# AidaDSP/aidadsp-lv2

Measured on AMD Instinct MI355X. Metric: audio samples/sec (48 kHz mono, many streams), higher is better.
Workload: dtype f32; 1 GPU; cfg2: LSTM-32 amp model, 1024 streams/GPU x 256-frame blocks, full run() chain, TTL-default controls; streams_per_gpu=1024, frames=256, kernel=k_lstm_pipe4<32>

## Files before the change

aidadsp-lv2_amd/csrc/aidax_device.h:

```cpp
#pragma once

#include <hip/hip_runtime.h>

#include <cfloat>

#include "aidax_layout.h"

namespace aidax {

__device__ __forceinline__ float dpp_row_shr1(float v)
{
    return __builtin_bit_cast(float, __builtin_amdgcn_update_dpp(0, __builtin_bit_cast(int, v), 0x111, 0xf, 0xf, true));
}

template <int CTRL, int ROW_MASK>
__device__ __forceinline__ float dpp_take(float v)
{
    return __builtin_bit_cast(float, __builtin_amdgcn_update_dpp(0, __builtin_bit_cast(int, v), CTRL, ROW_MASK, 0xf, ROW_MASK == 0xf));
}

__device__ __forceinline__ float wave_sum(float v)
{
    v = v + dpp_take<0xB1, 0xf>(v);
    v = v + dpp_take<0x4E, 0xf>(v);
    v = v + dpp_take<0x141, 0xf>(v);
    v = v + dpp_take<0x140, 0xf>(v);
    v = v + dpp_take<0x142, 0xa>(v);
    v = v + dpp_take<0x143, 0xc>(v);
    return __builtin_bit_cast(float, __builtin_amdgcn_readlane(__builtin_bit_cast(int, v), 63));
}

template <int N>
__device__ __forceinline__ void fmac_row_ror(float& acc, float h, float w)
{
    static_assert(N >= 1 && N <= 15, "rotation within a row of 16 lanes");
    asm volatile("v_fmac_f32_dpp %0, %1, %2 row_ror:%3 row_mask:0xf bank_mask:0xf" : "+v"(acc) : "v"(h), "v"(w), "n"(N));
}

#define AIDAX_ROR1(N, W) "v_fmac_f32_dpp %0, %1, %" #W " row_ror:" #N " row_mask:0xf bank_mask:0xf\n\t"
__device__ __forceinline__ void fmac_row_ror_1_15(float& a0, float h, const float* w)
{
    asm volatile(AIDAX_ROR1(1, 2) AIDAX_ROR1(2, 3) AIDAX_ROR1(3, 4) AIDAX_ROR1(4, 5) AIDAX_ROR1(5, 6) AIDAX_ROR1(6, 7) AIDAX_ROR1(7, 8)
                 AIDAX_ROR1(8, 9) AIDAX_ROR1(9, 10) AIDAX_ROR1(10, 11) AIDAX_ROR1(11, 12) AIDAX_ROR1(12, 13) AIDAX_ROR1(13, 14)
                 AIDAX_ROR1(14, 15) AIDAX_ROR1(15, 16)
                 : "+v"(a0)
                 : "v"(h), "v"(w[1]), "v"(w[2]), "v"(w[3]), "v"(w[4]), "v"(w[5]), "v"(w[6]), "v"(w[7]), "v"(w[8]), "v"(w[9]),
                   "v"(w[10]), "v"(w[11]), "v"(w[12]), "v"(w[13]), "v"(w[14]), "v"(w[15]));
}
#undef AIDAX_ROR1

typedef float aidax_f32x2 __attribute__((ext_vector_type(2)));
#define AIDAX_PKA(ACC, W, HQ) "v_pk_fma_f32 %" #ACC ", %" #W ", %" #HQ ", %" #ACC " op_sel_hi:[1,0,1]\n\t"
#define AIDAX_PKB(ACC, W, HQ) "v_pk_fma_f32 %" #ACC ", %" #W ", %" #HQ ", %" #ACC " op_sel:[0,1,0] op_sel_hi:[1,1,1]\n\t"
#define AIDAX_PKA0(ACC, W, HQ) "v_pk_fma_f32 %" #ACC ", %" #W ", %" #HQ ", 0 op_sel_hi:[1,0,0]\n\t"
#define AIDAX_PKB0(ACC, W, HQ) "v_pk_fma_f32 %" #ACC ", %" #W ", %" #HQ ", 0 op_sel:[0,1,0] op_sel_hi:[1,1,0]\n\t"
__device__ __forceinline__ aidax_f32x2 pk_fma_lds16(aidax_f32x2 pA, const aidax_f32x2* w, const aidax_f32x2* hq)
{
    aidax_f32x2 pB, pC, pD;
    asm volatile(AIDAX_PKA(0, 4, 20) AIDAX_PKB0(1, 5, 20) AIDAX_PKA0(2, 6, 21) AIDAX_PKB0(3, 7, 21)
                 AIDAX_PKA(0, 8, 22) AIDAX_PKB(1, 9, 22) AIDAX_PKA(2, 10, 23) AIDAX_PKB(3, 11, 23)
                 AIDAX_PKA(0, 12, 24) AIDAX_PKB(1, 13, 24) AIDAX_PKA(2, 14, 25) AIDAX_PKB(3, 15, 25)
                 AIDAX_PKA(0, 16, 26) AIDAX_PKB(1, 17, 26) AIDAX_PKA(2, 18, 27) AIDAX_PKB(3, 19, 27)
                 "v_pk_add_f32 %0, %0, %1\n\t"
                 "v_pk_add_f32 %2, %2, %3"
                 : "+v"(pA), "=&v"(pB), "=&v"(pC), "=&v"(pD)
                 : "v"(w[0]), "v"(w[1]), "v"(w[2]), "v"(w[3]), "v"(w[4]), "v"(w[5]), "v"(w[6]), "v"(w[7]), "v"(w[8]), "v"(w[9]), "v"(w[10]),
                   "v"(w[11]), "v"(w[12]), "v"(w[13]), "v"(w[14]), "v"(w[15]),
                   "v"(hq[0]), "v"(hq[1]), "v"(hq[2]), "v"(hq[3]), "v"(hq[4]), "v"(hq[5]), "v"(hq[6]), "v"(hq[7]));
    return pA + pC;
}
#undef AIDAX_PKA
#undef AIDAX_PKB
#undef AIDAX_PKA0
#undef AIDAX_PKB0

struct Pair { float lo, hi; };

__device__ __forceinline__ Pair share_halves(float v)
{
    const unsigned u = __builtin_bit_cast(unsigned, v);
    const auto r = __builtin_amdgcn_permlane32_swap(u, u, false, false);
    const unsigned r0 = r[0], r1 = r[1];
    return { __builtin_bit_cast(float, r0), __builtin_bit_cast(float, r1) };
}

__device__ __forceinline__ Pair share_rows(float v)
{
    const unsigned u = __builtin_bit_cast(unsigned, v);
    const auto r = __builtin_amdgcn_permlane16_swap(u, u, false, false);
    const unsigned r0 = r[0], r1 = r[1];
    return { __builtin_bit_cast(float, r0), __builtin_bit_cast(float, r1) };
}

__device__ __forceinline__ float fast_sigmoid(float v)
{
    const float e = __builtin_amdgcn_exp2f(v * -1.44269504088896340736f);
    return __builtin_amdgcn_rcpf(1.0f + e);
}

constexpr float kNegLog2e = -1.44269504088896340736f;
__device__ __forceinline__ float sigmoid_pre(float v_scaled)
{
    return __builtin_amdgcn_rcpf(1.0f + __builtin_amdgcn_exp2f(v_scaled));
}


constexpr float kTanhP[7] = { 0.9999999933888696f, 0.13084010352004496f, 0.003103956503888039f, 1.1154311501654368e-05f,
                              -2.0225239996482085e-08f, 5.277955823366522e-11f, -8.488730763828322e-14f };
constexpr float kTanhQ[4] = { 1.0f, 0.46417337453820245f, 0.02449517952619233f, 0.00025461456545097517f };
constexpr float kTanhClamp = 0x1.f9b3c2p+2f;
__device__ __forceinline__ float tanh_rat_clamp(float v) { return __builtin_fminf(__builtin_fmaxf(v, -kTanhClamp), kTanhClamp); }
template <bool kUFirst = false>
__device__ __forceinline__ float tanh_rat(float v)
{
    const float x = tanh_rat_clamp(v);
    const float u = x * x;
#ifndef AIDAX_TANH_PLAIN
    typedef float f32x2_t __attribute__((ext_vector_type(2)));
    const f32x2_t uu = { u, u };
    auto step = [&](f32x2_t pq, f32x2_t c) { return kUFirst ? __builtin_elementwise_fma(uu, pq, c) : __builtin_elementwise_fma(pq, uu, c); };
    f32x2_t pq = { kTanhP[6], kTanhQ[3] };
    pq = step(pq, f32x2_t{ kTanhP[5], kTanhQ[2] });
    pq = step(pq, f32x2_t{ kTanhP[4], kTanhQ[1] });
    pq = step(pq, f32x2_t{ kTanhP[3], kTanhQ[0] });
    float pp = pq.x;
    pp = __builtin_fmaf(pp, u, kTanhP[2]);
    pp = __builtin_fmaf(pp, u, kTanhP[1]);
    pp = __builtin_fmaf(pp, u, kTanhP[0]);
    return (pp * x) * __builtin_amdgcn_rcpf(pq.y);
#endif
    float p = kTanhP[6];
    p = __builtin_fmaf(p, u, kTanhP[5]);
    p = __builtin_fmaf(p, u, kTanhP[4]);
    p = __builtin_fmaf(p, u, kTanhP[3]);
    p = __builtin_fmaf(p, u, kTanhP[2]);
    p = __builtin_fmaf(p, u, kTanhP[1]);
    p = __builtin_fmaf(p, u, kTanhP[0]);
    float q = kTanhQ[3];
    q = __builtin_fmaf(q, u, kTanhQ[2]);
    q = __builtin_fmaf(q, u, kTanhQ[1]);
    q = __builtin_fmaf(q, u, kTanhQ[0]);
    return (p * x) * __builtin_amdgcn_rcpf(q);
}

__device__ __forceinline__ float tanh_exp(float v)
{
    const float e = __builtin_amdgcn_exp2f(v * 2.88539008177792681472f);
    return __builtin_fmaf(-2.0f, __builtin_amdgcn_rcpf(1.0f + e), 1.0f);
}

__device__ __forceinline__ float tanh_exp_pre(float v_scaled)
{
    return __builtin_fmaf(-2.0f, __builtin_amdgcn_rcpf(1.0f + __builtin_amdgcn_exp2f(v_scaled)), 1.0f);
}

struct ExpRamp {
    float mem, coef, tc;
    __device__ __forceinline__ void arm(float m, float target, float c)
    {
        mem = m; coef = c; tc = target * (1.f - c);
    }
    __device__ __forceinline__ float next() { mem = mem * coef + tc; return mem; }
};

__device__ __forceinline__ float lin_next(float& mem, float target, float step)
{
    const float y0 = mem;
    const float dy = target - y0;
    mem = y0 + __builtin_copysignf(__builtin_fminf(__builtin_fabsf(dy), __builtin_fabsf(step)), dy);
    return mem;
}

__device__ __forceinline__ bool eq_stage_transparent(double a0, double a1, double a2, double b1, double b2, double z1, double z2)
{
    return a0 == 1.0 && a1 == b1 && a2 == b2 && z1 == 0.0 && z2 == 0.0;
}
__device__ __forceinline__ float eq_skip_sample(float y, float& p)
{
    const float o = y + p;
    p = p + (y - y);
    return o;
}

struct ChainPass {
    int K, gain_lane;
    bool active;
    double a0, a1, a2, b1, b2, z1, z2;
    ExpRamp g;
    bool eq_skip;
    float eq_p;
};

template <int DST_STRIDE, bool CHECK>
__device__ __forceinline__ void chain_step(ChainPass& c, int stage, bool run, bool writer, float head, float& carry,
                                           float* dst, int s, int n)
{
    const float from_left = dpp_row_shr1(carry);
    const float x = stage == 0 ? head : from_left;
    const int idx = s - stage;
    if (!CHECK || (run && idx >= 0 && idx < n)) {
        const double xd = x;
        const double yd = xd * c.a0 + c.z1;
        c.z1 = xd * c.a1 + c.z2 - c.b1 * yd;
        c.z2 = xd * c.a2 - c.b2 * yd;
        float y = c.active ? (float)yd : x;
        const float gm = c.g.next();
        if (stage == c.gain_lane) y = y * gm;
        carry = y;
        if (writer) dst[idx * DST_STRIDE] = y;
    }
}

template <int DST_STRIDE = 1>
__device__ __forceinline__ void chain_sweep(ChainPass& c, int stage, bool run, int depth, const float* src, float* dst, int n)
{
    const double z1o = c.z1, z2o = c.z2;
    const bool writer = run && stage == c.K - 1;
    float carry = 0.f;
    const int steps = n + depth - 1;
    const int fill = depth - 1 < steps ? depth - 1 : steps;
    float head_next = src[0];
    int s = 0;
    for (; s < fill; ++s) {
        const float head = head_next;
        head_next = src[s + 1 < n ? s + 1 : n - 1];
        chain_step<DST_STRIDE, true>(c, stage, run, writer, head, carry, dst, s, n);
        __builtin_amdgcn_wave_barrier();
    }
    for (; s < n; ++s) {
        const float head = head_next;
        head_next = src[s + 1 < n ? s + 1 : n - 1];
        chain_step<DST_STRIDE, false>(c, stage, run, writer, head, carry, dst, s, n);
        __builtin_amdgcn_wave_barrier();
    }
    for (; s < steps; ++s) {
        chain_step<DST_STRIDE, true>(c, stage, run, writer, head_next, carry, dst, s, n);
        __builtin_amdgcn_wave_barrier();
    }
    if (!run || !c.active) { c.z1 = z1o; c.z2 = z2o; }
}

#ifndef AIDAX_CHAIN_BLOCK
#define AIDAX_CHAIN_BLOCK 8
#endif
constexpr int kChainBlock = AIDAX_CHAIN_BLOCK;

template <bool PLAIN, int B = kChainBlock, int HL = kWave, bool EQSKIP = false>
__device__ __forceinline__ void chain_macro_step(ChainPass& c, ExpRamp& g, int stage, bool run, bool last,
                                                 float* row, float* hand, int M, int m, int lane)
{
    const int j = m - stage;
    if (run && j >= 0 && j < M) {
        const float g_fixed = g.mem;
        const float* src = stage == 0 ? row + B * j : hand + (((m - 1) & 1) * HL + lane - 1) * B;
        float* dst = last ? row + B * j : hand + ((m & 1) * HL + lane) * B;
        float v[B];
#pragma unroll
        for (int q = 0; q < B / 4; ++q) {
            const float4 t = *reinterpret_cast<const float4*>(src + 4 * q);
            v[4 * q] = t.x; v[4 * q + 1] = t.y; v[4 * q + 2] = t.z; v[4 * q + 3] = t.w;
        }
#pragma unroll
        for (int i = 0; i < B; ++i) {
            const float x = v[i];
            const double xd = x;
            const double yd = xd * c.a0 + c.z1;
            c.z1 = xd * c.a1 + c.z2 - c.b1 * yd;
            c.z2 = xd * c.a2 - c.b2 * yd;
// ... 316 lines not shown
```

aidadsp-lv2_amd/csrc/aidax_kernels.hip:

```cpp
#include <hip/hip_runtime.h>
#include <hip/hip_ext.h>

#include <cfloat>

#include <mutex>
#include "aidax_device.h"
#include "aidax_kernels.h"
#include "aidax_layout.h"

namespace aidax {

template <int H, bool ROTP = true>
struct LstmCell {
    static constexpr LaneMap M = lstm_map(H);
    static constexpr int S = M.S, SLOTS = M.slots, NU = M.NU, GPL = M.GPL;
    static constexpr int PACK = lstm_pack_regs(H);
    static constexpr int STATE = 2 * H;
    static constexpr bool ROT4 = ROTP && lstm_rot4(H);
    static constexpr int KW = lstm_row_weights(H, ROT4);

    float w[NU][GPL][KW];
    typedef float f32x2 __attribute__((ext_vector_type(2)));
    f32x2 wl2[16];
    float wx[NU][GPL][kMaxInputs];
    float bias[NU][GPL];
    float wd[NU], bd;
    float aka[GPL], akb[GPL];
    float c[NU], h[NU];
    int part, slot;
#ifdef AIDAX_PIPE_TRACE
    unsigned long long ts6 = 0;
    unsigned long long ts[6];
#define PT_STAMP(k) do { if constexpr (TR) { __builtin_amdgcn_sched_barrier(0); ts[k] = __builtin_amdgcn_s_memtime(); __builtin_amdgcn_sched_barrier(0); } } while (0)
#else
#define PT_STAMP(k) do { } while (0)
#endif
    static constexpr int kStatePart = S == 2 ? 1 : 0;
    static constexpr bool ROT = ROTP && lstm_rot2(H);
    static constexpr int kPackOffset = (!ROTP && lstm_has_alt_pack(H)) ? lstm_alt_pack_offset(H) : 0;

    __device__ __forceinline__ void load(const float* __restrict__ wbase, const float* __restrict__ st, int lane)
    {
        const float* __restrict__ wp = wbase + kPackOffset;
        part = lane / SLOTS;
        slot = lane % SLOTS;
        int r = 0;
#pragma unroll
        for (int m = 0; m < NU; ++m)
#pragma unroll
            for (int e = 0; e < GPL; ++e) {
#pragma unroll
                for (int k = 0; k < KW; ++k) w[m][e][k] = wp[(r++) * kWave + lane];
#pragma unroll
                for (int i = 0; i < kMaxInputs; ++i) wx[m][e][i] = wp[(r++) * kWave + lane];
                bias[m][e] = wp[(r++) * kWave + lane];
            }
#pragma unroll
        for (int m = 0; m < NU; ++m) wd[m] = wp[(r++) * kWave + lane];
        bd = wp[(r++) * kWave + lane];
        if constexpr (ROTP && lstm_rot2(H)) {
            constexpr int kRow = KW + kMaxInputs + 1;
#pragma unroll
            for (int k = 0; k < 16; ++k) wl2[k] = f32x2{ wp[(16 + k) * kWave + lane], wp[(kRow + 16 + k) * kWave + lane] };
        }
#pragma unroll
        for (int e = 0; e < GPL; ++e) {
            const bool is_tanh = (part + S * e) == 2;
            aka[e] = is_tanh ? 1.f : 0.5f;
            akb[e] = is_tanh ? 0.f : 0.5f;
        }
#pragma unroll
        for (int m = 0; m < NU; ++m) {
            const int j = slot + m * SLOTS;
            h[m] = j < H ? st[j] : 0.f;
            c[m] = j < H ? st[H + j] : 0.f;
        }
    }

    __device__ __forceinline__ void store(float* __restrict__ st) const
    {
#pragma unroll
        for (int m = 0; m < NU; ++m) {
            const int j = slot + m * SLOTS;
            if (part == kStatePart && j < H) { st[j] = h[m]; st[H + j] = c[m]; }
        }
    }

    __device__ __forceinline__ void publish_h(float* hbuf) const
    {
#pragma unroll
        for (int m = 0; m < NU; ++m) {
            const int j = slot + m * SLOTS;
            if constexpr (S == 2 && !ROT) {
                if (j < H) hbuf[part == kStatePart ? j : H] = h[m];
            } else {
                if (j < H) hbuf[j] = h[m];
            }
        }
    }

    static constexpr int HID = H;

    __device__ __forceinline__ float dense_partial() const
    {
        float d = 0.f;
#pragma unroll
        for (int m = 0; m < NU; ++m) d = __builtin_fmaf(wd[m], h[m], d);
        return d;
    }

    template <int NI = kMaxInputs, int WINDOW = 0, bool TR = false>
    __device__ __forceinline__ void step(float x0, float x1, float x2, const float* hprev, float* hout)
    {
        PT_STAMP(0);
        float acc[NU][GPL];
#pragma unroll
        for (int m = 0; m < NU; ++m)
#pragma unroll
            for (int e = 0; e < GPL; ++e) {
                float a = bias[m][e];
                a = __builtin_fmaf(wx[m][e][0], x0, a);
                if constexpr (NI >= 2) a = __builtin_fmaf(wx[m][e][1], x1, a);
                if constexpr (NI >= 3) a = __builtin_fmaf(wx[m][e][2], x2, a);
                acc[m][e] = a;
            }
        if constexpr (ROT4) {
            const float hr = h[0];
            float a0 = __builtin_fmaf(w[0][0][0], hr, acc[0][0]);
            fmac_row_ror_1_15(a0, hr, w[0][0]);
            acc[0][0] = a0;
            (void)hprev;
        } else if constexpr (ROT) {
            const float4* hv = reinterpret_cast<const float4*>(hprev + 16 * (1 - ((slot >> 4) & 1)));
            const float4 q0 = hv[0], q1 = hv[1], q2 = hv[2], q3 = hv[3];
            __builtin_amdgcn_sched_barrier(0);
            const float hr = h[0];
            float a0 = acc[0][0], a1 = acc[0][1];
            a0 = __builtin_fmaf(w[0][0][0], hr, a0);
            a1 = __builtin_fmaf(w[0][1][0], hr, a1);
            fmac_row_ror_1_15(a0, hr, w[0][0]);
            fmac_row_ror_1_15(a1, hr, w[0][1]);
            __builtin_amdgcn_s_waitcnt(0xc07f);
            PT_STAMP(1);
            const f32x2 hq[8] = { f32x2{ q0.x, q0.y }, f32x2{ q0.z, q0.w }, f32x2{ q1.x, q1.y }, f32x2{ q1.z, q1.w },
                                  f32x2{ q2.x, q2.y }, f32x2{ q2.z, q2.w }, f32x2{ q3.x, q3.y }, f32x2{ q3.z, q3.w } };
            const f32x2 a01 = pk_fma_lds16(f32x2{ a0, a1 }, wl2, hq);
            acc[0][0] = a01.x; acc[0][1] = a01.y;
            PT_STAMP(2);
        } else {
        const float4* hv = reinterpret_cast<const float4*>(hprev);
#pragma unroll
        for (int k4 = 0; k4 < H / 4; ++k4) {
            const float4 q = hv[k4];
#pragma unroll
            for (int m = 0; m < NU; ++m)
#pragma unroll
                for (int e = 0; e < GPL; ++e) {
                    float a = acc[m][e];
                    a = __builtin_fmaf(w[m][e][4 * k4 + 0], q.x, a);
                    a = __builtin_fmaf(w[m][e][4 * k4 + 1], q.y, a);
                    a = __builtin_fmaf(w[m][e][4 * k4 + 2], q.z, a);
                    a = __builtin_fmaf(w[m][e][4 * k4 + 3], q.w, a);
                    acc[m][e] = a;
                }
            if constexpr (WINDOW > 0) { if ((k4 + 1) % WINDOW == 0) __builtin_amdgcn_sched_barrier(0); }
        }
        }
        __builtin_amdgcn_wave_barrier();
#pragma unroll
        for (int m = 0; m < NU; ++m) {
            float act[GPL];
#pragma unroll
            for (int e = 0; e < GPL; ++e) {
                if constexpr (S == 1) {
                    act[e] = e == 2 ? tanh_rat<ROT>(acc[m][e]) : sigmoid_pre(acc[m][e]);
                } else if (S == 2 && e == 0) {
                    act[e] = sigmoid_pre(acc[m][e]);
                } else {
                    act[e] = __builtin_fmaf(tanh_rat<ROT>(acc[m][e]), aka[e], akb[e]);
                }
            }
            PT_STAMP(3);
            float gi_gg, gf, go;
            if constexpr (S == 1) {
                gi_gg = act[0] * act[2]; gf = act[1]; go = act[3];
            } else if constexpr (S == 2) {
                const float ig = act[0] * act[1];
                const auto r = __builtin_amdgcn_permlane32_swap(__builtin_bit_cast(unsigned, acc[m][1]), __builtin_bit_cast(unsigned, ig), false, false);
                const unsigned r0 = r[0];
                gi_gg = __builtin_bit_cast(float, r0); gf = act[0]; go = act[1];
            } else {
                const Pair p = share_halves(act[0]);
                const Pair lo = share_rows(p.lo), hi = share_rows(p.hi);
                gi_gg = lo.lo * hi.lo; gf = lo.hi; go = hi.hi;
            }
            const float cn = __builtin_fmaf(gf, c[m], gi_gg);
            c[m] = cn;
#ifdef AIDAX_TANHC_EXP
            const float hn = go * tanh_exp(cn);
#else
            const float hn = go * tanh_rat<ROT>(cn);
#endif
            if constexpr (ROT) h[m] = share_halves(hn).hi;
            else h[m] = hn;
        }
        PT_STAMP(4);
        publish_h(hout);
        __builtin_amdgcn_wave_barrier();
        PT_STAMP(5);
    }
};

template <int H>
struct GruCell {
    static constexpr LaneMap M = gru_map(H);
    static constexpr int S = M.S, SLOTS = M.slots, NU = M.NU;
    static constexpr int KS = H / S;
    static constexpr int PACK = gru_pack_regs(H);
    static constexpr int STATE = H;
#ifdef AIDAX_PIPE_TRACE
    unsigned long long ts6 = 0, ts[6] = { 0, 0, 0, 0, 0, 0 };
#endif
    static_assert(KS % 4 == 0, "K slice must stay float4 aligned");

    float w[NU][3][KS];
    float wx[NU][3][kMaxInputs];
    float bias[NU][3];
    float bn1[NU];
    float wd[NU], bd;
    float h[NU];
    int part, slot;

    __device__ __forceinline__ void load(const float* __restrict__ wp, const float* __restrict__ st, int lane)
    {
        part = lane / SLOTS;
        slot = lane % SLOTS;
        int r = 0;
#pragma unroll
        for (int m = 0; m < NU; ++m)
#pragma unroll
            for (int e = 0; e < 3; ++e) {
#pragma unroll
                for (int k = 0; k < KS; ++k) w[m][e][k] = wp[(r++) * kWave + lane];
#pragma unroll
                for (int i = 0; i < kMaxInputs; ++i) wx[m][e][i] = wp[(r++) * kWave + lane];
                bias[m][e] = wp[(r++) * kWave + lane];
            }
#pragma unroll
        for (int m = 0; m < NU; ++m) bn1[m] = wp[(r++) * kWave + lane];
#pragma unroll
        for (int m = 0; m < NU; ++m) wd[m] = wp[(r++) * kWave + lane];
        bd = wp[(r++) * kWave + lane];
#pragma unroll
        for (int m = 0; m < NU; ++m) {
            const int j = slot + m * SLOTS;
            h[m] = j < H ? st[j] : 0.f;
        }
    }

    __device__ __forceinline__ void store(float* __restrict__ st) const
    {
#pragma unroll
        for (int m = 0; m < NU; ++m) {
            const int j = slot + m * SLOTS;
            if (part == 0 && j < H) st[j] = h[m];
        }
    }

    __device__ __forceinline__ void publish_h(float* hbuf) const
    {
#pragma unroll
        for (int m = 0; m < NU; ++m) {
            const int j = slot + m * SLOTS;
            if (j < H) hbuf[j] = h[m];
        }
    }

    static constexpr int HID = H;

    __device__ __forceinline__ float dense_partial() const
    {
        float d = 0.f;
#pragma unroll
        for (int m = 0; m < NU; ++m) d = __builtin_fmaf(wd[m], h[m], d);
        return d;
    }

    __device__ __forceinline__ static float unit_sum(float v)
    {
        if constexpr (S == 1) return v;
        else if constexpr (S == 2) { const Pair p = share_halves(v); return p.lo + p.hi; }
        else { const Pair p = share_halves(v); const float t = p.lo + p.hi; const Pair q = share_rows(t); return q.lo + q.hi; }
    }

    template <int NI = kMaxInputs, int WINDOW = 0, bool TR = false>
    __device__ __forceinline__ void step(float x0, float x1, float x2, const float* hprev, float* hout)
    {
        float ax[NU][3], ar[NU][3];
#pragma unroll
        for (int m = 0; m < NU; ++m)
#pragma unroll
            for (int e = 0; e < 3; ++e) {
                float a = bias[m][e];
                a = __builtin_fmaf(wx[m][e][0], x0, a);
                if constexpr (NI >= 2) a = __builtin_fmaf(wx[m][e][1], x1, a);
                if constexpr (NI >= 3) a = __builtin_fmaf(wx[m][e][2], x2, a);
                ax[m][e] = a;
                ar[m][e] = e == 2 ? bn1[m] : 0.f;
            }
        const float4* hv = reinterpret_cast<const float4*>(hprev + part * KS);
#pragma unroll
        for (int k4 = 0; k4 < KS / 4; ++k4) {
            const float4 q = hv[k4];
#pragma unroll
            for (int m = 0; m < NU; ++m)
#pragma unroll
                for (int e = 0; e < 3; ++e) {
                    float a = ar[m][e];
                    a = __builtin_fmaf(w[m][e][4 * k4 + 0], q.x, a);
                    a = __builtin_fmaf(w[m][e][4 * k4 + 1], q.y, a);
                    a = __builtin_fmaf(w[m][e][4 * k4 + 2], q.z, a);
                    a = __builtin_fmaf(w[m][e][4 * k4 + 3], q.w, a);
                    ar[m][e] = a;
                }
            if constexpr (WINDOW > 0) { if ((k4 + 1) % WINDOW == 0) __builtin_amdgcn_sched_barrier(0); }
        }
        __builtin_amdgcn_wave_barrier();
#pragma unroll
        for (int m = 0; m < NU; ++m) {
            const float zp = unit_sum(ax[m][0] + ar[m][0]);
            const float rp = unit_sum(ax[m][1] + ar[m][1]);
            const float nh = unit_sum(ar[m][2]);
            const float z = sigmoid_pre(zp);
            const float r = sigmoid_pre(rp);
            const float pre = __builtin_fmaf(r, nh, ax[m][2]);
            const float n = tanh_exp_pre(pre);
            h[m] = __builtin_fmaf(z, h[m] - n, n);
        }
        publish_h(hout);
        __builtin_amdgcn_wave_barrier();
    }
};

template <class Cell, bool HasCell>
__device__ __forceinline__ void stream_body(const LaunchArgs& a, float* smem)
{
    const int lane = threadIdx.x;
    const int s = blockIdx.x;
    const int n = (int)a.n_frames;

    if constexpr (HasCell) {
        if (a.mode != MODE_CHAIN) {
            float* hbuf = smem;
            Cell cell;
            float* nnst = a.nn + (size_t)s * a.nn_stride;
            cell.load(a.wpack, nnst, lane);
            cell.publish_h(hbuf);
            __builtin_amdgcn_wave_barrier();
            StreamState* stp = a.st + s;
            float p1 = stp->p_mem[0], p2 = stp->p_mem[1];
            const float t1 = stp->p_tgt[0], t2 = stp->p_tgt[1], s1 = stp->p_step[0], s2 = stp->p_step[1];
            for (int t = 0; t < n; ++t) {
                float x = 0.f, q1 = 0.f, q2 = 0.f;
                if (a.mode == MODE_NN_ONLY) {
                    x = a.in[(size_t)t * a.input_size];
                    if (a.input_size >= 2) q1 = a.in[(size_t)t * a.input_size + 1];
                    if (a.input_size >= 3) q2 = a.in[(size_t)t * a.input_size + 2];
                } else {
                    if (a.input_size >= 2) q1 = lin_next(p1, t1, s1);
                    if (a.input_size >= 3) q2 = lin_next(p2, t2, s2);
                }
                x = x * a.in_gain;
// ... 390 lines not shown
                    }
                }
            }
        } else {
            if (p >= 2 && !(AIDAX_TUNE(a) & 524288)) {
                const int base = (p - 2) * kSB;
                const int cnt = n - base < kSB ? n - base : kSB;
                const int tl = lane < cnt ? lane : cnt - 1;
                const float xin = xq[((p - 2) % 3) * kStage + tl];
                float o = xin;
                if (net_on) {
                    asm volatile("" ::: "memory");
                    const float4* row = reinterpret_cast<const float4*>(hh + ((base + tl) & (kRing - 1)) * HS);
                    const float4* w4 = reinterpret_cast<const float4*>(wdl);
                    float y = wdl[H];
#pragma unroll 2
                    for (int k4 = 0; k4 < H / 4; ++k4) {
                        const float4 w = w4[k4];
                        const float4 hv = row[k4];
                        y = __builtin_fmaf(w.x, hv.x, y);
                        y = __builtin_fmaf(w.y, hv.y, y);
                        y = __builtin_fmaf(w.z, hv.z, y);
                        y = __builtin_fmaf(w.w, hv.w, y);
                    }
                    const float xg = xin * m_in_gain();
                    o = m_skip() ? xg + y : y;
                    o = o * m_out_gain();
                }
                if (lane < cnt) qb[lane] = o;
                __builtin_amdgcn_wave_barrier();
                const bool first_stage = p == 2, last_stage = p == n_sub + 1;
                const bool q_run = lane < cp.K, q_writer = lane == cp.K - 1;
                if (first_stage) {
                    for (int t = 0; t < cnt; ++t) {
                        chain_step<1, true>(cp, lane, q_run, q_writer, qb[t], q_carry, inbuf, base + t, n);
                        __builtin_amdgcn_wave_barrier();
                    }
                } else {
                    float head_next = qb[0];
                    for (int t = 0; t < cnt; ++t) {
                        const float head = head_next;
                        head_next = qb[t + 1 < cnt ? t + 1 : t];
                        chain_step<1, false>(cp, lane, q_run, q_writer, head, q_carry, inbuf, base + t, n);
                        __builtin_amdgcn_wave_barrier();
                    }
                }
                if (last_stage)
                    for (int t = cnt; t < cnt + cp.K - 1; ++t) {
                        chain_step<1, true>(cp, lane, q_run, q_writer, 0.f, q_carry, inbuf, base + t, n);
                        __builtin_amdgcn_wave_barrier();
                    }
                const int hi = last_stage ? n : base + cnt - (cp.K - 1);
                for (int i = q_done + lane; i < hi; i += kWave) out_row[i] = inbuf[i];
                if (hi > q_done) q_done = hi;
            }
        }
#ifdef AIDAX_PIPE_TRACE
        if (wave == 1 && lane == 0 && p < 18) stg_tr[2 * p + 1] = (uint32_t)(clock64() - tr_c0);
#endif
        __syncthreads();
    }
#ifdef AIDAX_PIPE_TRACE
    if (wave == 1 && lane == 0) stg_tr[36] = (uint32_t)(clock64() - tr_c0);
#endif

    if (wave == 0) {
        if (lane < cp.K) { st.z[slot][0] = cp.z1; st.z[slot][1] = cp.z2; }
        if (lane == 0) {
            st.pre_mem = cp.g.mem;
            st.pre_tgt = pre_tgt;
            st.pending = pending;
            if (net_on) {
                st.p_mem[0] = p_mem[0]; st.p_mem[1] = p_mem[1];
                st.p_tgt[0] = p_tgt[0]; st.p_tgt[1] = p_tgt[1];
                st.p_step[0] = p_step[0]; st.p_step[1] = p_step[1];
            }
        }
    } else if (wave == 1) {
        if (net_on) cell.store(nnst);
#ifdef AIDAX_PIPE_TRACE
        if constexpr (H == 32) {
            asm volatile("s_waitcnt vmcnt(0)" ::: "memory");
            if (lane == 0) {
#pragma unroll
                for (int k = 0; k < 6; ++k) out_row[8 + k] = __builtin_bit_cast(float, (uint32_t)(cell.ts[k] - cell.ts[0]));
                out_row[14] = __builtin_bit_cast(float, (uint32_t)(cell.ts6 - cell.ts[0]));
            }
            if (lane < 37) out_row[16 + lane] = __builtin_bit_cast(float, stg_tr[lane]);
        }
#endif
    } else {
        if (lane >= cp.K || !cp.active) { cp.z1 = q_z1o; cp.z2 = q_z2o; }
        if (lane < cp.K) { st.z[slot][0] = cp.z1; st.z[slot][1] = cp.z2; }
#ifdef AIDAX_TEST_HOOKS
        if (lane == 0) st.pad = (uint32_t)cp.K;
#endif
        if (lane == cp.K - 1) { st.master_mem = cp.g.mem; st.master_tgt = master_tgt; }
        post_done_word(a, lane);
#ifdef AIDAX_PIPE_TRACE
        asm volatile("s_waitcnt vmcnt(0)" ::: "memory");
        if (lane == 0) {
            out_row[0] = __builtin_bit_cast(float, (uint32_t)(tr_w0 & 0xffffffffu));
            out_row[1] = __builtin_bit_cast(float, (uint32_t)(wall_clock64() & 0xffffffffu));
            out_row[2] = __builtin_bit_cast(float, (uint32_t)(clock64() - tr_c0));
            out_row[3] = __builtin_bit_cast(float, (uint32_t)__builtin_amdgcn_s_getreg((31 << 11) | (0 << 6) | 4));
            out_row[4] = __builtin_bit_cast(float, (uint32_t)__builtin_amdgcn_s_getreg((3 << 11) | (0 << 6) | 20));
        }
#endif
    }
}

template <int H>
__global__ __launch_bounds__(kPipeWaves * kWave) void k_lstm_pipe(LaunchArgs a)
{
    extern __shared__ __attribute__((aligned(16))) float smem[];
    stream_body_pipe<LstmCell<H>>(a, smem);
}

template <int H>
__global__ __launch_bounds__(kPipeWaves * kWave) void k_gru_pipe(LaunchArgs a)
{
    extern __shared__ __attribute__((aligned(16))) float smem[];
    stream_body_pipe<GruCell<H>>(a, smem);
}

template <int H>
__global__ __launch_bounds__(kPipeWaves * kWave) void k_lstm_pipe_bank(LaunchArgs a)
{
    extern __shared__ __attribute__((aligned(16))) float smem[];
    stream_body_pipe<LstmCell<H>, true>(a, smem);
}

template <int H>
__global__ __launch_bounds__(kPipeWaves * kWave) void k_gru_pipe_bank(LaunchArgs a)
{
    extern __shared__ __attribute__((aligned(16))) float smem[];
    stream_body_pipe<GruCell<H>, true>(a, smem);
}


constexpr int kP4Streams = 4;
constexpr int kP4Helpers = 1;
constexpr int kP4Waves = kP4Streams + kP4Helpers;
constexpr int kP4ChainLanes = 12 * kP4Streams;
constexpr int kP4HandFloats = 2 * kP4ChainLanes * kStChainBlockP4;
__host__ __device__ constexpr size_t pipe4_lds_floats(int H, int n_frames, bool conditioned)
{
    return (size_t)kP4Streams * n_frames + (size_t)kP4Streams * kRing * pipe_row_stride(H) + kP4HandFloats + (size_t)(H + 4) + 8
         + 5 * kWave
         + (conditioned ? (size_t)2 * kP4Streams * n_frames : 0) ;
}
typedef __attribute__((address_space(3))) int p4_lds_int;
typedef int p4_i2 __attribute__((ext_vector_type(2)));
typedef __attribute__((address_space(3))) p4_i2 p4_lds_i2;
__device__ __forceinline__ int p4_peek(const int* w)
{
    const int v = *(const volatile p4_lds_int*)(const p4_lds_int*)(w);
    asm volatile("s_waitcnt lgkmcnt(0)" ::: "memory");
    return __builtin_amdgcn_readfirstlane(v);
}
__device__ __forceinline__ void p4_post(int* w, int v, int lane)
{
    asm volatile("" ::: "memory");
    if (lane == 0) *(volatile p4_lds_int*)(p4_lds_int*)(w) = v;
    asm volatile("" ::: "memory");
}

template <class Cell, bool kCond>
__device__ __forceinline__ void stream_body_pipe4(const LaunchArgs& a, float* smem)
{
    constexpr int H = Cell::HID;
    constexpr int HS = pipe_row_stride(H);
    constexpr int B = kStChainBlockP4;
    const int lane = threadIdx.x & 63;
    const int wave = __builtin_amdgcn_readfirstlane((int)(threadIdx.x >> 6));
    const int s0 = kP4Streams * blockIdx.x;
    const int n = (int)a.n_frames;
    const int NT = n / kSB;
#ifdef AIDAX_P4_TRACE
#define P4_STAMP(k) do { __builtin_amdgcn_sched_barrier(0); tr[k] = __builtin_amdgcn_s_memrealtime(); __builtin_amdgcn_sched_barrier(0); } while (0)
    unsigned long long tr[8] = {0, 0, 0, 0, 0, 0, 0, 0};
    P4_STAMP(0);
#else
#define P4_STAMP(k) do { } while (0)
#endif
    float* rows = smem;
    float* hh = rows + kP4Streams * n;
    float* hand = hh + kP4Streams * kRing * HS;
    float* wdl = hand + kP4HandFloats;
    int* prog = reinterpret_cast<int*>(wdl + H + 4);
    float* hstate = reinterpret_cast<float*>(prog + 8);
    float* prow = hstate + 5 * kWave;
    const int I = kCond ? (int)a.input_size : 1;

    int Kp = 1;
#ifdef AIDAX_P4_BARRIER
    int Kq = 1;
#endif
    uint32_t fw[kP4Streams];
#pragma unroll
    for (int j = 0; j < kP4Streams; ++j) {
        const int jc = s0 + j < (int)a.n_streams ? s0 + j : (int)a.n_streams - 1;
        const uint32_t f = a.ctl[jc].flags;
        fw[j] = s0 + j < (int)a.n_streams ? f : 0u;
        if ((f & CTL_EQ_PRE) && s0 + j < (int)a.n_streams) Kp = 6;
#ifdef AIDAX_P4_BARRIER
        if ((f & CTL_EQ_POST) && s0 + j < (int)a.n_streams) Kq = 6;
#endif
    }
    const int d1 = Kp / 2 + 1;
#ifdef AIDAX_P4_BARRIER
    const int T = (n / B - 1 + (Kq - 1) + 2 * (d1 + 1)) / 2 + 1;
#endif

    if (wave < kP4Streams) {
        const int s = s0 + wave;
        const int sc = s < (int)a.n_streams ? s : (int)a.n_streams - 1;
        float* nnst = a.nn + (size_t)sc * a.nn_stride;
        float* hj = hh + wave * kRing * HS;
        const float* row = rows + wave * n;
        Cell cell;
        if (!(AIDAX_TUNE(a) & 1)) __builtin_amdgcn_s_setprio(3);
        cell.load(a.wpack, nnst, lane);
        P4_STAMP(1);
        const uint32_t fl = wave == 0 ? fw[0] : wave == 1 ? fw[1] : wave == 2 ? fw[2] : fw[3];
        const bool net = (fl & (CTL_ENABLED | CTL_NET_ON)) == (CTL_ENABLED | CTL_NET_ON);
        cell.publish_h(hj + (kRing - 1) * HS);
        __syncthreads();
        P4_STAMP(2);
#ifndef AIDAX_P4_BARRIER
        if (!net) { p4_post(prog + 2 + wave, NT, lane); return; }
#endif
#ifdef AIDAX_P4_BARRIER
        for (int tick = 0; tick < T; ++tick) {
            const int t = tick - d1;
            for (int i = 0; i < wave * ((AIDAX_TUNE(a) >> 24) & 3); ++i) asm volatile("s_nop 15");
            if (t >= 0 && t < NT) {
#else
        for (int i = 0; i < wave * ((AIDAX_TUNE(a) >> 24) & 15); ++i) asm volatile("s_nop 15");
        p4_i2 ahead = p4_i2{ 0, 0 };
        for (int t = 0; t < NT; ++t) {
            if (ahead.x <= t || ahead.y < t - 1)
                while (p4_peek(prog) <= t || p4_peek(prog + 1) < t - 1) __builtin_amdgcn_s_sleep(1);
#ifdef AIDAX_P4_TRACE
            if (t == 0) P4_STAMP(3);
            if (t == 1) P4_STAMP(4);
            if (t == NT - 1) P4_STAMP(5);
            if (wave == 0 && t < 32) {
                __builtin_amdgcn_sched_barrier(0);
                const unsigned long long now = __builtin_amdgcn_s_memrealtime();
                if (lane == 0) reinterpret_cast<unsigned long long*>(hstate)[8 + t] = now;
                __builtin_amdgcn_sched_barrier(0);
            }
#endif
            {
#endif
                const int base = t * kSB;
                const float* hprev = hj + ((base + kRing - 1) & (kRing - 1)) * HS;
                float* hcur = hj + (base & (kRing - 1)) * HS;
                const float* xs = row + base;
                float xr[kSB];
                asm volatile(".p2align 6");
                auto fetch_x = [&](int q) {
                    const float4 v = reinterpret_cast<const float4*>(xs)[q];
                    xr[4 * q] = v.x; xr[4 * q + 1] = v.y;
                    xr[4 * q + 2] = v.z; xr[4 * q + 3] = v.w;
                };
                fetch_x(0);
                if constexpr (!kCond) {
#pragma unroll
                    for (int f = 0; f < kSB; ++f) {
                        if ((f & 3) == 1 && f / 4 + 1 < kSB / 4) fetch_x(f / 4 + 1);
#ifndef AIDAX_P4_BARRIER
                        if (f == kSB - 4) ahead = *(const volatile p4_lds_i2*)(const p4_lds_i2*)(prog);
#endif
                        cell.template step<1>(xr[f], 0.f, 0.f, f == 0 ? hprev : hcur + (f - 1) * HS, hcur + f * HS);
                    }
                } else {
                    const float* p1s = prow + (wave * 2 + 0) * n + base;
                    const float* p2s = prow + (wave * 2 + 1) * n + base;
                    float p1r[kSB], p2r[kSB];
                    auto fetch_p = [&](int q) {
                        const float4 u = reinterpret_cast<const float4*>(p1s)[q];
                        const float4 w = reinterpret_cast<const float4*>(p2s)[q];
                        p1r[4 * q] = u.x; p1r[4 * q + 1] = u.y; p1r[4 * q + 2] = u.z; p1r[4 * q + 3] = u.w;
                        p2r[4 * q] = w.x; p2r[4 * q + 1] = w.y; p2r[4 * q + 2] = w.z; p2r[4 * q + 3] = w.w;
                    };
                    fetch_p(0);
#pragma unroll
                    for (int f = 0; f < kSB; ++f) {
                        if ((f & 3) == 1 && f / 4 + 1 < kSB / 4) { fetch_x(f / 4 + 1); fetch_p(f / 4 + 1); }
#ifndef AIDAX_P4_BARRIER
                        if (f == kSB - 4) ahead = *(const volatile p4_lds_i2*)(const p4_lds_i2*)(prog);
#endif
                        cell.template step<3>(xr[f], p1r[f], I >= 3 ? p2r[f] : 0.f, f == 0 ? hprev : hcur + (f - 1) * HS, hcur + f * HS);
                    }
                }
            }
#ifdef AIDAX_P4_BARRIER
            __syncthreads();
#else
            p4_post(prog + 2 + wave, t + 1, lane);
#endif
        }
        P4_STAMP(6);
        cell.store(nnst);
#ifdef AIDAX_P4_TRACE
        P4_STAMP(7);
        {
            unsigned long long mine = 0;
#pragma unroll
            for (int k = 0; k < 8; ++k) if (lane == k) mine = tr[k];
            if (wave == 0 && lane < 8) reinterpret_cast<unsigned long long*>(hstate)[lane] = mine;
        }
#endif
        return;
    }

    const int hq = wave - kP4Streams;
    const int j = lane < kP4ChainLanes ? lane / 12 : kP4Streams - 1;
    const int r = lane - 12 * (lane / 12);
    const bool isQ = r >= 6;
    const int stage = isQ ? r - 6 : r;
    const bool there = s0 + j < (int)a.n_streams;
    const int sj = there ? s0 + j : (int)a.n_streams - 1;
    const StreamCtl& ctl = a.ctl[sj];
    StreamState& st = a.st[sj];
    const int slot = isQ ? post_slot(stage) : pre_slot(stage);
    float4 r0 = float4{0.f, 0.f, 0.f, 0.f}, r1 = r0, r2 = r0, r3 = r0;
    if (kP4Helpers == 1 && n == 256) {
        const bool t1 = s0 + 1 < (int)a.n_streams, t2 = s0 + 2 < (int)a.n_streams, t3 = s0 + 3 < (int)a.n_streams;
        r0 = reinterpret_cast<const float4*>(a.in + (size_t)s0 * n)[lane];
        r1 = reinterpret_cast<const float4*>(a.in + (size_t)(t1 ? s0 + 1 : s0) * n)[lane];
        r2 = reinterpret_cast<const float4*>(a.in + (size_t)(t2 ? s0 + 2 : s0) * n)[lane];
        r3 = reinterpret_cast<const float4*>(a.in + (size_t)(t3 ? s0 + 3 : s0) * n)[lane];
    } else if (kP4Helpers == 1 && n < 256) {
        const int have4 = ((int)a.n_streams - s0 < kP4Streams ? (int)a.n_streams - s0 : kP4Streams) * (n / 4);
        const float4* g4 = reinterpret_cast<const float4*>(a.in + (size_t)s0 * n);
        const int i0 = lane, i1 = kWave + lane, i2 = 2 * kWave + lane, i3 = 3 * kWave + lane;
        r0 = g4[i0 < have4 ? i0 : 0];
        r1 = g4[i1 < have4 ? i1 : 0];
        r2 = g4[i2 < have4 ? i2 : 0];
        r3 = g4[i3 < have4 ? i3 : 0];
    }
    static_assert(H + 1 <= kWave, "the Dense's weights and bias: a lane each");
    const float* wd_nat = a.wpack + (size_t)Cell::PACK * kWave;
    const float wdv = wd_nat[lane < H + 1 ? lane : 0];
    ChainPass c;
    chain_load(c, ctl, st, slot, false);
    const uint32_t flags = ctl.flags;
    uint32_t pending = st.pending;
    float pre_mem = st.pre_mem, master_mem = st.master_mem, pre_tgt = st.pre_tgt, master_tgt = st.master_tgt;
    const float ctl_pre_target = ctl.pre_target, ctl_master_target = ctl.master_target, ctl_pre_coef = ctl.pre_coef, ctl_master_coef = ctl.master_coef;
    const int dj = lane >> 4, df = lane & 15;
    const uint32_t fdj = a.ctl[s0 + dj < (int)a.n_streams ? s0 + dj : (int)a.n_streams - 1].flags;
    static_assert(kP4Helpers == 1, "the PARAM lanes' state is not handed from helper to helper");
    const bool plane = kCond && lane >= kP4ChainLanes && lane < kP4ChainLanes + 2 * kP4Streams;
    const int jp = plane ? (lane - kP4ChainLanes) >> 1 : 0, ip = lane & 1;
    const bool there_p = s0 + jp < (int)a.n_streams;
    const int sp = there_p ? s0 + jp : (int)a.n_streams - 1;
    float pm = 0.f, pt = 0.f, ps = 0.f, p_nt = 0.f, p_den = 1.f;
    uint32_t p_flags = 0, p_pending = 0;
    if constexpr (kCond) {
        pm = a.st[sp].p_mem[ip]; pt = a.st[sp].p_tgt[ip]; ps = a.st[sp].p_step[ip];
        p_nt = a.ctl[sp].p_target[ip]; p_den = a.ctl[sp].p_den;
        p_flags = a.ctl[sp].flags; p_pending = a.st[sp].pending;
    }
    if (kP4Helpers == 1 && n == 256) {
        reinterpret_cast<float4*>(rows)[lane] = r0;
        reinterpret_cast<float4*>(rows + n)[lane] = r1;
        reinterpret_cast<float4*>(rows + 2 * n)[lane] = r2;
        reinterpret_cast<float4*>(rows + 3 * n)[lane] = r3;
    } else if (kP4Helpers == 1 && n < 256) {
        float4* l4 = reinterpret_cast<float4*>(rows);
        const int i0 = lane, i1 = kWave + lane, i2 = 2 * kWave + lane, i3 = 3 * kWave + lane;
        if (i0 < n) l4[i0] = r0;
        if (i1 < n) l4[i1] = r1;
        if (i2 < n) l4[i2] = r2;
        if (i3 < n) l4[i3] = r3;
    } else {
        for (int jj = hq; jj < kP4Streams; jj += kP4Helpers) {
            if (s0 + jj >= (int)a.n_streams) break;
            const float4* src = reinterpret_cast<const float4*>(a.in + (size_t)(s0 + jj) * n);
            float4* dst = reinterpret_cast<float4*>(rows + jj * n);
            for (int i = lane; i < n / 4; i += kWave) dst[i] = src[i];
        }
    }
    if (hq == 0 && lane < H + 1) wdl[lane] = wdv;
    const bool live = there && (flags & CTL_ENABLED) != 0;
    const bool netj = live && (flags & CTL_NET_ON) != 0;
    if (pending & PEND_ACTIVATE) { pre_mem = pre_tgt; master_mem = master_tgt; pending &= ~PEND_ACTIVATE; }
    pre_tgt = ctl_pre_target;
    if (live) master_tgt = ctl_master_target;
    bool skipj = false;
#ifndef AIDAX_P4_BARRIER
    {
        const unsigned long long flat = __builtin_amdgcn_ballot_w64(eq_stage_transparent(c.a0, c.a1, c.a2, c.b1, c.b2, c.z1, c.z2));
        skipj = ((flat >> (12 * j + 7)) & 31u) == 31u && (flags & (CTL_EQ_POST | CTL_EQ_BANDPASS)) == CTL_EQ_POST
             && !(AIDAX_TUNE(a) & kTuneEqFull);
    }
#endif
    const int Kpj = (flags & CTL_EQ_PRE) ? 6 : 1, Kqj = (flags & CTL_EQ_POST) && !skipj ? 6 : 1;
#ifndef AIDAX_P4_BARRIER
    const int Kq = __builtin_amdgcn_ballot_w64(there && lane < kP4ChainLanes && Kqj == 6) != 0 ? 6 : 1;
    const int T = (n / B - 1 + (Kq - 1) + 2 * (d1 + 1)) / 2 + 1;
#endif
    c.K = isQ ? Kqj : Kpj;
    c.gain_lane = isQ ? Kqj - 1 : 0;
    c.eq_skip = skipj && isQ && stage == 0;
    c.eq_p = 0.f;
    c.active = stage == 0 ? (flags & (isQ ? CTL_DC_ON : CTL_LPF_ON)) != 0 : ((flags & CTL_EQ_BANDPASS) ? slot == BQ_MID : true);
    c.g.arm(isQ ? master_mem : pre_mem, isQ ? master_tgt : pre_tgt, isQ ? ctl_master_coef : ctl_pre_coef);
    const bool run = lane < kP4ChainLanes && stage < c.K && live;
    const double z1o = c.z1, z2o = c.z2;
    ExpRamp g = c.g;
    const bool is_gain = stage == c.gain_lane;
    if (!is_gain) { g.mem = 1.f; g.coef = 1.f; g.tc = 0.f; }
    const bool last = stage == c.K - 1;
    const bool fussy = run && (!c.active || g.mem * g.coef + g.tc != g.mem);
    const bool plain = __builtin_amdgcn_ballot_w64(fussy) == 0;
    const int m0 = isQ ? 2 * (d1 + 1) : 0;
    float* myrow = rows + j * n;
// ... 594 lines not shown
```

Baseline: 4.674 billion samples/s.

## Pin LSTM-32 pipe4 frame state to fixed registers and prefetch next-frame input gates

Adds a packed-frame path for the LSTM-32 pipe4 kernel. Each frame's recurrent head is done with hand-written DPP row-rotate FMACs on pinned VGPR pairs. The next frame's input-projection FMA is folded into the current frame's LDS dot-product asm. The h output is shared with a packed multiply plus permlane32 swap, and the tanh clamp switches to med3. The aim is to cut per-frame serial latency on the recurrence, at the cost of fragile hard-coded register constraints (v[2:3], v[4:5], v[6:7]) that may clash with compiler allocation.

```diff
diff --git a/aidadsp-lv2_amd/csrc/aidax_device.h b/aidadsp-lv2_amd/csrc/aidax_device.h
--- a/aidadsp-lv2_amd/csrc/aidax_device.h
+++ b/aidadsp-lv2_amd/csrc/aidax_device.h
@@ -69,10 +69,74 @@
                    "v"(hq[0]), "v"(hq[1]), "v"(hq[2]), "v"(hq[3]), "v"(hq[4]), "v"(hq[5]), "v"(hq[6]), "v"(hq[7]));
     return pA + pC;
 }
+
+#define AIDAX_ROR2(A, N, W) "v_fmac_f32_dpp " A ", %3, %" #W " row_ror:" #N " row_mask:0xf bank_mask:0xf\n\t"
+#define AIDAX_ROR2_ROW(A, W0, W1, W2, W3, W4, W5, W6, W7, W8, W9, W10, W11, W12, W13, W14) \
+    AIDAX_ROR2(A, 1, W0) AIDAX_ROR2(A, 2, W1) AIDAX_ROR2(A, 3, W2) AIDAX_ROR2(A, 4, W3) AIDAX_ROR2(A, 5, W4) AIDAX_ROR2(A, 6, W5) \
+    AIDAX_ROR2(A, 7, W6) AIDAX_ROR2(A, 8, W7) AIDAX_ROR2(A, 9, W8) AIDAX_ROR2(A, 10, W9) AIDAX_ROR2(A, 11, W10) AIDAX_ROR2(A, 12, W11) \
+    AIDAX_ROR2(A, 13, W12) AIDAX_ROR2(A, 14, W13) AIDAX_ROR2(A, 15, W14)
+#define AIDAX_HEAD_P4(PAIR, LO, HI)                                                                                                        \
+    asm volatile("v_pk_fma_f32 " PAIR ", %1, %2, " PAIR " op_sel_hi:[0,1,1]\n\t"                                                          \
+                 AIDAX_ROR2_ROW(LO, 4, 5, 6, 7, 8, 9, 10, 11, 12, 13, 14, 15, 16, 17, 18)                                                  \
+                 AIDAX_ROR2_ROW(HI, 19, 20, 21, 22, 23, 24, 25, 26, 27, 28, 29, 30, 31, 32, 33)                                            \
+                 : "+{" PAIR "}"(a01)                                                                                                      \
+                 : "v"(hp), "v"(w00), "v"(hp.x),                                                                                           \
+                   "v"(w0[1]), "v"(w0[2]), "v"(w0[3]), "v"(w0[4]), "v"(w0[5]), "v"(w0[6]), "v"(w0[7]), "v"(w0[8]), "v"(w0[9]), "v"(w0[10]), \
+                   "v"(w0[11]), "v"(w0[12]), "v"(w0[13]), "v"(w0[14]), "v"(w0[15]),                                                        \
+                   "v"(w1[1]), "v"(w1[2]), "v"(w1[3]), "v"(w1[4]), "v"(w1[5]), "v"(w1[6]), "v"(w1[7]), "v"(w1[8]), "v"(w1[9]), "v"(w1[10]), \
+                   "v"(w1[11]), "v"(w1[12]), "v"(w1[13]), "v"(w1[14]), "v"(w1[15]))
+template <int PAR>
+__device__ __forceinline__ aidax_f32x2 lstm32_head_p4(aidax_f32x2 a01, aidax_f32x2 hp, aidax_f32x2 w00, const float* w0, const float* w1)
+{
+    if constexpr (PAR == 0) AIDAX_HEAD_P4("v[2:3]", "v2", "v3");
+    else AIDAX_HEAD_P4("v[6:7]", "v6", "v7");
+    return a01;
+}
+#undef AIDAX_HEAD_P4
+#undef AIDAX_ROR2_ROW
+#undef AIDAX_ROR2
+#define AIDAX_LDS16_P4(PAIR, XSEL)                                                                                                         \
+    asm volatile(AIDAX_PKA(0, 5, 21) AIDAX_PKB0(1, 6, 21) AIDAX_PKA0(2, 7, 22) AIDAX_PKB0(3, 8, 22)                                       \
+                 AIDAX_PKA(0, 9, 23) AIDAX_PKB(1, 10, 23) AIDAX_PKA(2, 11, 24) AIDAX_PKB(3, 12, 24)                                        \
+                 AIDAX_PKA(0, 13, 25) AIDAX_PKB(1, 14, 25) AIDAX_PKA(2, 15, 26) AIDAX_PKB(3, 16, 26)                                       \
+                 AIDAX_PKA(0, 17, 27) AIDAX_PKB(1, 18, 27) AIDAX_PKA(2, 19, 28) AIDAX_PKB(3, 20, 28)                                       \
+                 "v_pk_add_f32 %0, %0, %1\n\t"                                                                                            \
+                 "v_pk_add_f32 %2, %2, %3\n\t"                                                                                            \
+                 "v_pk_fma_f32 " PAIR ", %29, %30, %31 " XSEL "\n\t"                                                                      \
+                 "v_pk_add_f32 %2, %0, %2"                                                                                                \
+                 : "+v"(pA), "=&v"(pB), "=&v"(pC), "=&v"(pD), "=&{" PAIR "}"(an)                                                           \
+                 : "v"(w[0]), "v"(w[1]), "v"(w[2]), "v"(w[3]), "v"(w[4]), "v"(w[5]), "v"(w[6]), "v"(w[7]), "v"(w[8]), "v"(w[9]), "v"(w[10]), \
+                   "v"(w[11]), "v"(w[12]), "v"(w[13]), "v"(w[14]), "v"(w[15]),                                                             \
+                   "v"(hq[0]), "v"(hq[1]), "v"(hq[2]), "v"(hq[3]), "v"(hq[4]), "v"(hq[5]), "v"(hq[6]), "v"(hq[7]),                         \
+                   "v"(xn), "v"(wx), "v"(b))
+template <int PARN>
+__device__ __forceinline__ aidax_f32x2 pk_fma_lds16_p4(aidax_f32x2 pA, const aidax_f32x2* w, const aidax_f32x2* hq,
+                                                       aidax_f32x2 xn, aidax_f32x2 wx, aidax_f32x2 b, aidax_f32x2& an)
+{
+    aidax_f32x2 pB, pC, pD;
+    if constexpr (PARN == 0) AIDAX_LDS16_P4("v[2:3]", "op_sel_hi:[0,1,1]");
+    else AIDAX_LDS16_P4("v[6:7]", "op_sel:[1,0,0] op_sel_hi:[1,1,1]");
+    return pC;
+}
+#undef AIDAX_LDS16_P4
 #undef AIDAX_PKA
 #undef AIDAX_PKB
 #undef AIDAX_PKA0
 #undef AIDAX_PKB0
+struct P4Frame { aidax_f32x2 hp, an; };
+__device__ __forceinline__ aidax_f32x2 lstm32_end_p4(float go, float t)
+{
+    typedef float f32x1_t __attribute__((ext_vector_type(1)));
+    const aidax_f32x2 g2 = __builtin_shufflevector(f32x1_t{ go }, f32x1_t{ go }, 0, -1);
+    const aidax_f32x2 t2 = __builtin_shufflevector(f32x1_t{ t }, f32x1_t{ t }, 0, -1);
+    aidax_f32x2 hp;
+    asm volatile("v_pk_mul_f32 v[4:5], %1, %2 op_sel_hi:[0,0]\n\t"
+                 "s_nop 1\n\t"
+                 "v_permlane32_swap_b32 v5, v4"
+                 : "={v[4:5]}"(hp)
+                 : "v"(g2), "v"(t2));
+    return hp;
+}
 
 struct Pair { float lo, hi; };
 
@@ -110,10 +174,11 @@
 constexpr float kTanhQ[4] = { 1.0f, 0.46417337453820245f, 0.02449517952619233f, 0.00025461456545097517f };
 constexpr float kTanhClamp = 0x1.f9b3c2p+2f;
 __device__ __forceinline__ float tanh_rat_clamp(float v) { return __builtin_fminf(__builtin_fmaxf(v, -kTanhClamp), kTanhClamp); }
-template <bool kUFirst = false>
+__device__ __forceinline__ float tanh_rat_clamp_med3(float v) { return __builtin_amdgcn_fmed3f(v, -kTanhClamp, kTanhClamp); }
+template <bool kUFirst = false, bool kClamped = false>
 __device__ __forceinline__ float tanh_rat(float v)
 {
-    const float x = tanh_rat_clamp(v);
+    const float x = kClamped ? v : tanh_rat_clamp(v);
     const float u = x * x;
 #ifndef AIDAX_TANH_PLAIN
     typedef float f32x2_t __attribute__((ext_vector_type(2)));
diff --git a/aidadsp-lv2_amd/csrc/aidax_kernels.hip b/aidadsp-lv2_amd/csrc/aidax_kernels.hip
--- a/aidadsp-lv2_amd/csrc/aidax_kernels.hip
+++ b/aidadsp-lv2_amd/csrc/aidax_kernels.hip
@@ -4,6 +4,7 @@
 #include <cfloat>
 
 #include <mutex>
+#include <type_traits>
 #include "aidax_device.h"
 #include "aidax_kernels.h"
 #include "aidax_layout.h"
@@ -100,6 +101,7 @@
     }
 
     static constexpr int HID = H;
+    static constexpr bool kPackedFrame = ROTP && lstm_rot2(H);
 
     __device__ __forceinline__ float dense_partial() const
     {
@@ -109,9 +111,11 @@
         return d;
     }
 
-    template <int NI = kMaxInputs, int WINDOW = 0, bool TR = false>
-    __device__ __forceinline__ void step(float x0, float x1, float x2, const float* hprev, float* hout)
+    static constexpr int kP4On = 1, kP4Odd = 2, kP4Next = 4, kP4First = 8;
+    template <int NI = kMaxInputs, int WINDOW = 0, bool TR = false, int kP4F = 0>
+    __device__ __forceinline__ void step(float x0, float x1, float x2, const float* hprev, float* hout, P4Frame* pf = nullptr, f32x2 xn = f32x2{ 0.f, 0.f })
     {
+        static_assert(!kP4F || (ROT && NI == 1 && NU == 1), "the packed frame is LSTM-32's with the audio as its one input");
         PT_STAMP(0);
         float acc[NU][GPL];
 #pragma unroll
@@ -130,6 +134,23 @@
             fmac_row_ror_1_15(a0, hr, w[0][0]);
             acc[0][0] = a0;
             (void)hprev;
+        } else if constexpr (ROT && kP4F != 0) {
+            constexpr int kPar = (kP4F & kP4Odd) ? 1 : 0;
+            const f32x2 wx2 = f32x2{ wx[0][0][0], wx[0][1][0] }, b2 = f32x2{ bias[0][0], bias[0][1] };
+            f32x2 a01 = pf->an;
+            if constexpr (kP4F & kP4First) a01 = __builtin_elementwise_fma(f32x2{ x0, x0 }, wx2, b2);
+            const float4* hv = reinterpret_cast<const float4*>(hprev + 16 * (1 - ((slot >> 4) & 1)));
+            const float4 q0 = hv[0], q1 = hv[1], q2 = hv[2], q3 = hv[3];
+            __builtin_amdgcn_sched_barrier(0);
+            a01 = lstm32_head_p4<kPar>(a01, pf->hp, f32x2{ w[0][0][0], w[0][1][0] }, w[0][0], w[0][1]);
+            __builtin_amdgcn_s_waitcnt(0xc07f);
+            PT_STAMP(1);
+            const f32x2 hq[8] = { f32x2{ q0.x, q0.y }, f32x2{ q0.z, q0.w }, f32x2{ q1.x, q1.y }, f32x2{ q1.z, q1.w },
+                                  f32x2{ q2.x, q2.y }, f32x2{ q2.z, q2.w }, f32x2{ q3.x, q3.y }, f32x2{ q3.z, q3.w } };
+            if constexpr (kP4F & kP4Next) a01 = pk_fma_lds16_p4<1 - kPar>(a01, wl2, hq, xn, wx2, b2, pf->an);
+            else a01 = pk_fma_lds16(a01, wl2, hq);
+            acc[0][0] = a01.x; acc[0][1] = a01.y;
+            PT_STAMP(2);
         } else if constexpr (ROT) {
             const float4* hv = reinterpret_cast<const float4*>(hprev + 16 * (1 - ((slot >> 4) & 1)));
             const float4 q0 = hv[0], q1 = hv[1], q2 = hv[2], q3 = hv[3];
@@ -176,6 +197,8 @@
                     act[e] = e == 2 ? tanh_rat<ROT>(acc[m][e]) : sigmoid_pre(acc[m][e]);
                 } else if (S == 2 && e == 0) {
                     act[e] = sigmoid_pre(acc[m][e]);
+                } else if constexpr (kP4F != 0) {
+                    act[e] = __builtin_fmaf(tanh_rat<true, true>(tanh_rat_clamp_med3(acc[m][e])), aka[e], akb[e]);
                 } else {
                     act[e] = __builtin_fmaf(tanh_rat<ROT>(acc[m][e]), aka[e], akb[e]);
                 }
@@ -197,11 +220,14 @@
             const float cn = __builtin_fmaf(gf, c[m], gi_gg);
             c[m] = cn;
 #ifdef AIDAX_TANHC_EXP
-            const float hn = go * tanh_exp(cn);
+            const float tc = tanh_exp(cn);
+            const float hn = go * tc;
 #else
-            const float hn = go * tanh_rat<ROT>(cn);
-#endif
-            if constexpr (ROT) h[m] = share_halves(hn).hi;
+            const float tc = tanh_rat<ROT>(cn);
+            const float hn = go * tc;
+#endif
+            if constexpr (ROT && kP4F != 0) { pf->hp = lstm32_end_p4(go, tc); h[m] = pf->hp.x; }
+            else if constexpr (ROT) h[m] = share_halves(hn).hi;
             else h[m] = hn;
         }
         PT_STAMP(4);
@@ -218,6 +244,7 @@
     static constexpr int KS = H / S;
     static constexpr int PACK = gru_pack_regs(H);
     static constexpr int STATE = H;
+    static constexpr bool kPackedFrame = false;
 #ifdef AIDAX_PIPE_TRACE
     unsigned long long ts6 = 0, ts[6] = { 0, 0, 0, 0, 0, 0 };
 #endif
@@ -914,6 +941,7 @@
 }
 typedef __attribute__((address_space(3))) int p4_lds_int;
 typedef int p4_i2 __attribute__((ext_vector_type(2)));
+typedef float p4_f32x2 __attribute__((ext_vector_type(2)));
 typedef __attribute__((address_space(3))) p4_i2 p4_lds_i2;
 __device__ __forceinline__ int p4_peek(const int* w)
 {
@@ -984,6 +1012,8 @@
         Cell cell;
         if (!(AIDAX_TUNE(a) & 1)) __builtin_amdgcn_s_setprio(3);
         cell.load(a.wpack, nnst, lane);
+        P4Frame pf;
+        if constexpr (Cell::kPackedFrame) { pf.hp = p4_f32x2{ cell.h[0], cell.h[0] }; pf.an = p4_f32x2{ 0.f, 0.f }; }
         P4_STAMP(1);
         const uint32_t fl = wave == 0 ? fw[0] : wave == 1 ? fw[1] : wave == 2 ? fw[2] : fw[3];
         const bool net = (fl & (CTL_ENABLED | CTL_NET_ON)) == (CTL_ENABLED | CTL_NET_ON);
@@ -1029,7 +1059,23 @@
                     xr[4 * q + 2] = v.z; xr[4 * q + 3] = v.w;
                 };
                 fetch_x(0);
-                if constexpr (!kCond) {
+                if constexpr (!kCond && Cell::kPackedFrame) {
+                    auto frame = [&](auto fc) {
+                        constexpr int f = decltype(fc)::value;
+                        constexpr int fn = f + 1 < kSB ? f + 1 : f;
+                        if ((f & 3) == 1 && f / 4 + 1 < kSB / 4) fetch_x(f / 4 + 1);
+#ifndef AIDAX_P4_BARRIER
+                        if (f == kSB - 4) ahead = *(const volatile p4_lds_i2*)(const p4_lds_i2*)(prog);
+#endif
+                        cell.template step<1, 0, false, Cell::kP4On | (f & 1 ? Cell::kP4Odd : 0) | (f + 1 < kSB ? Cell::kP4Next : 0) | (f == 0 ? Cell::kP4First : 0)>(
+                            xr[f], 0.f, 0.f, f == 0 ? hprev : hcur + (f - 1) * HS, hcur + f * HS, &pf, p4_f32x2{ xr[fn & ~1], xr[fn | 1] });
+                    };
+                    static_assert(kSB == 16, "sixteen frames to a tile");
+#define P4_FRAME(F) frame(std::integral_constant<int, F>{})
+                    P4_FRAME(0); P4_FRAME(1); P4_FRAME(2); P4_FRAME(3); P4_FRAME(4); P4_FRAME(5); P4_FRAME(6); P4_FRAME(7);
+                    P4_FRAME(8); P4_FRAME(9); P4_FRAME(10); P4_FRAME(11); P4_FRAME(12); P4_FRAME(13); P4_FRAME(14); P4_FRAME(15);
+#undef P4_FRAME
+                } else if constexpr (!kCond) {
 #pragma unroll
                     for (int f = 0; f < kSB; ++f) {
                         if ((f & 3) == 1 && f / 4 + 1 < kSB / 4) fetch_x(f / 4 + 1);
```

After: 4.682 billion samples/s, median of 6. No clear change (+0.2%).
